# desy-ml/cheetah

Hardware: AMD Instinct MI355X
Metric: particle-element-steps/sec at 1e6 particles, 100-elem linac (higher is better)
Workload: dtype f32; 1 GPU; C2: 100-element Drift+Quadrupole FODO, 1e6 particles per GPU, fp32, element-by-element tracking (no map merging) + global beam moments; elements=100, particles_per_gpu=1000000, parallelism=particle-shard x1, sigma_x_checked=True

## Files before the change

### cheetah_amd/_lib.py

```python

from __future__ import annotations

import ctypes
import os

import torch

_HERE = os.path.dirname(os.path.abspath(__file__))
LIB_PATH = os.path.join(_HERE, "libchx.so")

c_void_p, c_int, c_i64, c_double, c_size_t = (
    ctypes.c_void_p,
    ctypes.c_int,
    ctypes.c_int64,
    ctypes.c_double,
    ctypes.c_size_t,
)
c_i32_p = ctypes.POINTER(ctypes.c_int32)
c_u8_p = ctypes.POINTER(ctypes.c_uint8)
c_vpp = ctypes.POINTER(ctypes.c_void_p)
c_double_p = ctypes.POINTER(ctypes.c_double)


class ChxError(RuntimeError):
# ... 6 lines not shown
        ("ndim", ctypes.c_int32),
        ("cols", ctypes.c_int32 * 3),
        ("bins", ctypes.c_int32 * 3),
        ("grid_strides", ctypes.c_int64 * 3),
        ("grid_batch_stride", ctypes.c_int64),
        ("B", c_i64), ("Bx", c_i64), ("Bq", c_i64), ("Bs", c_i64), ("Be", c_i64),
        ("Bsc", c_i64), ("Bsh", c_i64), ("N", c_i64),
        ("dtype", ctypes.c_int32),
        ("abs_charge", ctypes.c_int32),
        ("x", c_void_p), ("charge", c_void_p), ("survival", c_void_p), ("extent", c_void_p),
        ("scale", c_void_p), ("shift", c_void_p), ("grid", c_void_p),
    ]


class LatticeScreen(ctypes.Structure):

    _fields_ = [
        ("rows", c_void_p), ("charges", c_void_p), ("survival", c_void_p), ("energy", c_void_p), ("s", c_void_p),
        ("image", c_void_p), ("image_bytes", c_i64), ("map", c_void_p), ("element_maps", c_void_p),
        ("mu", c_void_p), ("cov", c_void_p), ("geom", c_void_p), ("shift", c_void_p), ("total_charge", c_void_p),
        ("total_charge_out", c_void_p), ("width", ctypes.c_int32), ("height", ctypes.c_int32),
        ("mom_partials", c_void_p),
    ]


class Hist2dArgs(ctypes.Structure):

    _fields_ = [
        ("B", c_i64), ("Bx", c_i64), ("Bq", c_i64), ("Bs", c_i64), ("Bsh", c_i64), ("N", c_i64),
        ("nx", ctypes.c_int32), ("ny", ctypes.c_int32), ("dtype", ctypes.c_int32),
        ("x", c_void_p), ("charge", c_void_p), ("survival", c_void_p), ("shift", c_void_p),
        ("edges_x", c_void_p), ("edges_y", c_void_p), ("image", c_void_p),
    ]


SIGNATURES = {
    "chx_kind_num_params": (c_int, [c_int]),
    "chx_abi_version": (c_int, []),
    "chx_status_string": (ctypes.c_char_p, [c_int]),
    "chx_build_rmatrix": (c_int, [c_int, c_void_p, c_void_p, c_double, c_double, c_i64, c_i64, c_i64, c_int, c_void_p, c_void_p]),
    "chx_build_rmatrix_vjp": (c_int, [c_int, c_void_p, c_void_p, c_double, c_double, c_void_p, c_i64, c_i64, c_i64, c_int, c_void_p, c_void_p, c_void_p]),
    "chx_compose_maps": (c_int, [c_vpp, c_u8_p, c_i64, c_i64, c_int, c_void_p, c_void_p]),
    "chx_compose_maps_vjp_workspace_bytes": (c_size_t, [c_i64, c_i64]),
    "chx_compose_maps_vjp": (c_int, [c_vpp, c_u8_p, c_i64, c_i64, c_int, c_void_p, c_void_p, c_void_p, c_size_t, c_void_p]),
    "chx_compose_prefix": (c_int, [c_void_p, c_i64, c_i64, c_i64, c_int, c_void_p, c_void_p]),
    "chx_run_state_bytes": (c_size_t, [c_i64]),
    "chx_run_map": (c_int, [c_void_p, c_void_p, c_i64, c_void_p, c_double, c_double, c_int, c_void_p, c_size_t, c_void_p,
                            c_void_p, c_void_p, c_void_p]),
    "chx_run_track": (c_int, [c_void_p, c_void_p, c_i64, c_void_p, c_double, c_double, c_int, c_void_p, c_size_t, c_void_p,
                              c_void_p, c_i64, c_void_p, c_void_p, c_void_p]),
    "chx_apply_affine7": (c_int, [c_void_p, c_void_p, c_void_p, c_i64, c_i64, c_i64, c_i64, c_int, c_void_p]),
    "chx_apply_bwd_workspace_bytes": (c_size_t, [c_i64, c_i64]),
    "chx_apply_affine7_bwd": (c_int, [c_void_p, c_void_p, c_void_p, c_void_p, c_void_p, c_i64, c_i64, c_i64, c_i64, c_int, c_void_p, c_size_t, c_void_p]),
    "chx_track_elementwise": (c_int, [c_void_p, c_void_p, c_void_p, c_void_p, c_i64, c_i64, c_i64, c_i64, c_i64, c_int, c_void_p]),
    "chx_track_fused": (c_int, [c_void_p, c_void_p, c_void_p, c_i64, c_i64, c_i64, c_i64, c_i64, c_int, c_void_p]),
    "chx_cavity_coeffs": (c_int, [c_void_p, c_void_p, c_double, c_double, c_i64, c_i64, c_i64, c_int, c_void_p, c_void_p, c_void_p]),
    "chx_cavity_track": (c_int, [c_void_p, c_void_p, c_void_p, c_void_p, c_i64, c_i64, c_i64, c_int, c_void_p]),
    "chx_cavity_track_bwd": (c_int, [c_void_p, c_void_p, c_void_p, c_void_p, c_void_p, c_i64, c_i64, c_i64, c_int, c_void_p,
                                     c_size_t, c_void_p]),
    "chx_moments_workspace_bytes": (c_size_t, [c_i64, c_i64]),
    "chx_moment_sums": (c_int, [c_void_p, c_void_p, c_i64, c_i64, c_i64, c_i64, c_int, c_void_p, c_void_p, c_size_t, c_void_p]),
    "chx_moment_centred": (c_int, [c_void_p, c_void_p, c_void_p, c_i64, c_i64, c_i64, c_i64, c_int, c_void_p, c_void_p, c_size_t, c_void_p]),
    "chx_moment_finalize": (c_int, [c_void_p, c_void_p, c_i64, c_void_p, c_void_p]),
    "chx_moments": (c_int, [c_void_p, c_void_p, c_i64, c_i64, c_i64, c_i64, c_int, c_void_p, c_void_p, c_size_t, c_void_p]),
    "chx_moments_entry": (c_int, [c_void_p, c_void_p, c_i64, c_i64, c_i64, c_i64, c_int, c_void_p, c_int, c_int, c_void_p, c_void_p,
                                  c_size_t, c_void_p]),
    "chx_moments_bwd": (c_int, [c_void_p, c_void_p, c_void_p, c_void_p, c_i64, c_i64, c_i64, c_i64, c_int, c_void_p, c_void_p]),
    "chx_moments_bwd_w": (c_int, [c_void_p, c_void_p, c_void_p, c_void_p, c_i64, c_i64, c_i64, c_i64, c_int, c_void_p, c_void_p,
                                  c_void_p]),
    "chx_moments_mapped_bwd": (c_int, [c_void_p, c_void_p, c_void_p, c_i64, c_i64, c_i64, c_int, c_void_p, c_void_p]),
    "chx_moment_entry": (c_int, [c_void_p, c_i64, c_int, c_int, c_int, c_void_p, c_void_p]),
    "chx_moment_entry_mapped_bwd": (c_int, [c_void_p, c_void_p, c_int, c_int, c_void_p, c_void_p, c_i64, c_i64, c_i64, c_int,
                                            c_void_p, c_int, c_void_p]),
    "chx_cic_deposit": (c_int, [ctypes.POINTER(CicArgs), c_void_p]),
    "chx_cic_deposit_mapped": (c_int, [ctypes.POINTER(CicArgs), c_void_p, c_i64, c_void_p]),
    "chx_cic_sorted_workspace_bytes": (c_size_t, [ctypes.POINTER(CicArgs)]),
    "chx_cic_deposit_sorted": (c_int, [ctypes.POINTER(CicArgs), c_void_p, c_size_t, c_void_p]),
    "chx_cic_deposit_sorted_overwrite": (c_int, [ctypes.POINTER(CicArgs), c_void_p, c_size_t, c_void_p]),
    "chx_cic_indices": (c_int, [ctypes.POINTER(CicArgs), c_void_p, c_void_p, c_void_p]),
    "chx_cic_deposit_bwd": (c_int, [ctypes.POINTER(CicArgs), c_void_p, c_void_p, c_void_p, c_void_p]),
    "chx_hist2d": (c_int, [ctypes.POINTER(Hist2dArgs), c_void_p]),
    "chx_hist2d_indices": (c_int, [ctypes.POINTER(Hist2dArgs), c_void_p, c_void_p]),
    "chx_sc_igf_workspace_bytes": (c_size_t, [c_i64, c_i32_p]),
    "chx_sc_igf": (c_int, [c_void_p, c_void_p, c_i64, c_i32_p, c_int, c_void_p, c_i64, c_void_p, c_size_t, c_void_p]),
    "chx_sc_igf_from_table": (c_int, [c_void_p, c_i64, c_i32_p, c_int, c_void_p, c_i64, c_void_p]),
    "chx_sc_pruned_supported": (c_int, [c_i32_p, c_int]),
    "chx_sc_igf_table": (c_int, [c_void_p, c_void_p, c_i64, c_i32_p, c_int, c_void_p, c_void_p]),
    "chx_sc_green_workspace_bytes": (c_size_t, [c_i64, c_i32_p, c_int]),
    "chx_sc_green_fast_workspace_bytes": (c_size_t, [c_i64, c_i32_p, c_int]),
    "chx_sc_green_spectrum_fast": (c_int, [c_void_p, c_void_p, c_i64, c_i32_p, c_int, c_void_p, c_void_p, c_size_t, c_void_p]),
    "chx_sc_green_spectrum": (c_int, [c_void_p, c_i64, c_i32_p, c_int, c_void_p, c_void_p, c_size_t, c_void_p]),
    "chx_sc_convolve_workspace_bytes": (c_size_t, [c_i64, c_i32_p, c_int]),
    "chx_sc_convolve": (c_int, [c_void_p, c_void_p, c_void_p, c_i64, c_i32_p, c_int, c_void_p, c_void_p, c_size_t, c_void_p]),
    "chx_sc_fft_plan_create": (c_int, [c_i64, c_i32_p, c_int, c_vpp]),
    "chx_sc_fft_plan_destroy": (c_int, [c_void_p]),
    "chx_sc_fft_exec": (c_int, [c_void_p, c_int, c_void_p, c_void_p]),
    "chx_sc_spectral_mul": (c_int, [c_void_p, c_void_p, c_void_p, c_i64, c_i64, c_int, c_void_p]),
    "chx_sc_phi_halo_elements": (c_size_t, [c_i64, c_i32_p]),
    "chx_sc_convolve_halo": (c_int, [c_void_p, c_void_p, c_void_p, c_i64, c_i32_p, c_int, c_void_p, c_void_p, c_size_t, c_void_p]),
    "chx_sc_convolve_halo_after": (c_int, [c_void_p, c_void_p, c_void_p, c_i64, c_i32_p, c_int, c_void_p, c_void_p, c_size_t, c_void_p,
                                           c_void_p]),
    "chx_sc_gather_kick_phi": (c_int, [c_void_p, c_void_p, c_void_p, c_void_p, c_void_p, c_void_p, c_void_p, c_double, c_i64, c_i64,
                                       c_i64, c_i64, c_i32_p, c_int, c_void_p, c_i64, c_void_p, c_void_p]),
    "chx_sc_gradient": (c_int, [c_void_p, c_void_p, c_void_p, c_i64, c_i32_p, c_int, c_i64, c_int, c_void_p, c_void_p]),
    "chx_sc_gather_kick": (c_int, [c_void_p, c_void_p, c_void_p, c_void_p, c_void_p, c_void_p, c_double, c_i64, c_i64, c_i64, c_i64, c_i32_p, c_int, c_void_p, c_void_p]),
    "chx_sc_gather_kick_mapped": (c_int, [c_void_p, c_void_p, c_void_p, c_void_p, c_void_p, c_void_p, c_double, c_i64, c_i64, c_i64,
# ... 227 lines not shown
```

### cheetah_amd/_ops.py

```python

from __future__ import annotations

import ctypes
import weakref
import os

import torch

from . import _lib
from ._lib import CicArgs, Hist2dArgs, check

KIND = {
    "identity": 0, "drift": 1, "quadrupole": 2, "dipole": 3, "hcor": 4, "vcor": 5, "ccor": 6,
    "cavity_sw": 7, "cavity_tw": 8, "solenoid": 9, "undulator": 10,
}
NUM_PARAMS = [0, 1, 5, 9, 2, 2, 3, 4, 4, 4, 4]
MOM_NOUT = 29
CAV_NCOEF = 8


def dtype_code(dtype: torch.dtype) -> int:
    if dtype == torch.float32:
        return 0
    if dtype == torch.float64:
# ... 461 lines not shown
    root = _origin(source)
    copy._chx_origin = (weakref.ref(root), root._version, copy._version)


def _origin(t: torch.Tensor) -> torch.Tensor:
    while True:
        tag = getattr(t, "_chx_origin", None)
        if tag is None or tag[2] != t._version:
            return t
        src = tag[0]()
        if src is None or src._version != tag[1]:
            return t
        t = src


def apply_map(particles: torch.Tensor, tm: torch.Tensor) -> torch.Tensor:
    require_device(particles, tm)
    if tm.dtype != particles.dtype:
        raise RuntimeError(f"transfer map dtype {tm.dtype} does not match particle dtype {particles.dtype}")
    N = particles.shape[-2]
    batch_shape = bshapes(particles.shape[:-2], tm.shape[:-2])
    B = numel(batch_shape)
    x, _ = flat_bcast(particles, batch_shape, 2)
    R, _ = flat_bcast(tm, batch_shape, 2)
    x, R = aligned(x), R.contiguous()
    if x.requires_grad or R.requires_grad:
        out = Apply.apply(x, R, B).reshape(*batch_shape, N, 7)
        if not x.requires_grad and torch.is_grad_enabled():
            out._chx_lin = _LinearSource(_origin(particles), x, R, batch_shape, out._version)
        return out
    out = _apply_raw(x, R, B, x.shape[0], R.shape[0], N)
    return out.reshape(*batch_shape, N, 7)


def track_elementwise(particles, maps: torch.Tensor, fused: bool = False) -> torch.Tensor:
    require_device(particles, maps)
    if torch.is_grad_enabled() and (particles.requires_grad or maps.requires_grad):
        x = particles
        for e in range(maps.shape[0]):
            x = apply_map(x, maps[e] if maps.shape[1] > 1 else maps[e, 0])
        return x
    E, BR = maps.shape[0], maps.shape[1]
    N = particles.shape[-2]
    batch_shape = torch.broadcast_shapes(particles.shape[:-2], (BR,) if BR > 1 else ())
    B = numel(batch_shape)
    x, Bx = flat_bcast(particles, batch_shape, 2)
    x, maps = aligned(x), maps.contiguous()
    out = torch.empty((B, N, 7), dtype=x.dtype, device=x.device)
    lib = _lib.lib()
    if fused:
        check(lib.chx_track_fused(ptr(x), ptr(maps), ptr(out), E, B, Bx, BR, N, dtype_code(x.dtype), stream_ptr()),
              "chx_track_fused")
    else:
        check(lib.chx_track_elementwise(ptr(x), ptr(maps), ptr(out), None, E, B, Bx, BR, N,
                                        dtype_code(x.dtype), stream_ptr()), "chx_track_elementwise")
    return out.reshape(*batch_shape, N, 7)


def _cavity_coeffs_autograd(params, energy, mass_eV, n_charges, B):
    import math

    p = params.to(torch.float64).expand(B, 4)
    L, V, phi, freq = p[:, 0], p[:, 1], p[:, 2] * (math.pi / 180.0), p[:, 3]
    E0 = energy.to(torch.float64).expand(B)
    g0 = E0 / mass_eV
    ig2 = 1.0 / (g0 * g0)
    b0 = (1.0 - ig2).sqrt()
    cphi, sphi = phi.cos(), phi.sin()
    dEn = V * cphi * n_charges * -1.0
    E1 = E0 + dEn
    g1 = E1 / mass_eV
    b1 = (1.0 - 1.0 / (g1 * g1)).sqrt()
    k = 2.0 * math.pi * freq / 299792458.0
    gain = (dEn > 0).any()
    dg = V / mass_eV
    b03, b13, g03, g13 = b0**3, b1**3, g0**3, g1**3
    gd = g0 - g1
    gd = torch.where(gd == 0, torch.ones_like(gd), gd)
    T566_gain = L * (b03 * g03 - b13 * g13) / (2.0 * b0 * b13 * g0 * gd * g13)
    T556_gain = b0 * k * L * dg * g0 * (b13 * g13 + b0 * (g0 - g13)) * sphi / (b13 * g13 * gd * gd)
    T555_gain = b0 * b0 * k * k * L * dg / 2.0 * (
        dg * (2.0 * g0 * g13 * (b0 * b13 - 1.0) + g0 * g0 + 3.0 * g1 * g1 - 2.0) / (b13 * g13 * gd**3) * sphi * sphi
        - (g1 * g0 * (b1 * b0 - 1.0) + 1.0) / (b1 * g1 * gd * gd) * cphi)
    zero = torch.zeros_like(L)
    T566 = torch.where(gain, T566_gain, 1.5 * L * ig2 / b03)
    T556 = torch.where(gain, T556_gain, zero)
    T555 = torch.where(gain, T555_gain, zero)
    coeffs = torch.stack([E0 * b0 / (E1 * b1), V * b0 / (E1 * b1), b0 * k, phi, cphi, T566, T556, T555], dim=-1)
    return coeffs, E1.to(energy.dtype)


def cavity_coeffs(params, energy, mass_eV, n_charges, B):
    if params.requires_grad or energy.requires_grad:
        return _cavity_coeffs_autograd(params, energy, mass_eV, n_charges, B)
    coeffs = torch.empty((B, CAV_NCOEF), dtype=torch.float64, device=energy.device)
    e_out = torch.empty((B,), dtype=energy.dtype, device=energy.device)
    check(_lib.lib().chx_cavity_coeffs(ptr(params), ptr(energy), mass_eV, n_charges, B, params.shape[0],
                                       energy.shape[0], dtype_code(energy.dtype), ptr(coeffs), ptr(e_out),
                                       stream_ptr()), "chx_cavity_coeffs")
    return coeffs, e_out


def _cavity_track_raw(x, R, coeffs, B, N):
    out = torch.empty((B, N, 7), dtype=x.dtype, device=x.device)
    check(_lib.lib().chx_cavity_track(ptr(x), ptr(R), ptr(coeffs), ptr(out), B, x.shape[0], N,
                                      dtype_code(x.dtype), stream_ptr()), "chx_cavity_track")
    return out
# ... 753 lines not shown
```

### cheetah_amd/csrc/chx_apply.hip

```cpp
#include <cstdlib>
#include <type_traits>

#include "chx_common.h"
#include "chx_apply_tiles.h"
#include "chx_cic_dev.h"

namespace {

template <typename T> __device__ __forceinline__ T chx_fma(T a, T b, T c);
template <> __device__ __forceinline__ float chx_fma<float>(float a, float b, float c) { return fmaf(a, b, c); }
template <> __device__ __forceinline__ double chx_fma<double>(double a, double b, double c) { return fma(a, b, c); }

template <typename T>
__device__ __forceinline__ void apply7(const T* __restrict__ R, const T (&x)[7], T (&y)[7]) {
#pragma unroll
    for (int i = 0; i < 7; ++i) {
        T acc = R[i * 7] * x[0];
#pragma unroll
        for (int j = 1; j < 7; ++j) acc = chx_fma<T>(R[i * 7 + j], x[j], acc);
        y[i] = acc;
    }
}

template <typename T>
// ... 409 lines not shown
        int64_t wchunks = (8192 + wtiles - 1) / wtiles;
        if (wchunks > B) wchunks = B;
        int64_t wrows = (B + wchunks - 1) / wchunks;
        if (wrows < 8 && B >= 8) wrows = 8;
        wchunks = (B + wrows - 1) / wrows;
        if (wtiles > 0x7fffffffLL || wchunks > 65535) return CHX_ERR_INVALID_ARG;
        hipLaunchKernelGGL((apply_shared_wave_kernel<T, WPPT>), dim3((unsigned)wtiles, (unsigned)wchunks), dim3(CHX_BLOCK), 0, s,
                           (const T*)x_in, (const T*)R, (T*)x_out, B, N, wrows, (int)chx_aligned16(x_in));
    } else
        hipLaunchKernelGGL((apply_shared_kernel<T, PPT>), dim3((unsigned)tiles, (unsigned)chunks),
                           dim3(CHX_BLOCK), 0, s, (const T*)x_in, (const T*)R, (T*)x_out, B, N, rows,
                           (int)chx_aligned16(x_in), (int)chx_aligned16(x_out));
    CHX_CHECK_LAUNCH();
    return CHX_OK;
}

int check_common(const void* x_in, const void* R, const void* x_out, int64_t B, int64_t Bx,
                 int64_t BR, int64_t N, int dtype) {
    if (!x_in || !R || !x_out || B < 1 || N < 1) return CHX_ERR_INVALID_ARG;
    if (!chx_bcast_ok(Bx, B) || !chx_bcast_ok(BR, B)) return CHX_ERR_INVALID_ARG;
    if (dtype != CHX_F32 && dtype != CHX_F64) return CHX_ERR_DTYPE;
    const size_t esz = dtype == CHX_F32 ? 4 : 8;
    if ((reinterpret_cast<uintptr_t>(x_in) % esz) || (reinterpret_cast<uintptr_t>(x_out) % esz) ||
        (reinterpret_cast<uintptr_t>(R) % esz))
        return CHX_ERR_MISALIGNED;
    return CHX_OK;
}

}

extern "C" int chx_apply_affine7(const void* x_in, const void* R, void* x_out, int64_t B, int64_t Bx,
                                 int64_t BR, int64_t N, int dtype, void* stream) {
    int st = check_common(x_in, R, x_out, B, Bx, BR, N, dtype);
    if (st != CHX_OK) return st;
    hipStream_t s = (hipStream_t)stream;
    if (Bx == 1 && B > 1 && BR == B) {
        return dtype == CHX_F32 ? launch_shared<float>(x_in, R, x_out, B, N, s)
                                : launch_shared<double>(x_in, R, x_out, B, N, s);
    }
    return dtype == CHX_F32 ? launch_tiles<float, 0>(x_in, R, x_out, nullptr, B, Bx, BR, N, 1, s)
                            : launch_tiles<double, 0>(x_in, R, x_out, nullptr, B, Bx, BR, N, 1, s);
}

extern "C" int chx_track_fused(const void* x_in, const void* R, void* x_out, int64_t E, int64_t B,
                               int64_t Bx, int64_t BR, int64_t N, int dtype, void* stream) {
    int st = check_common(x_in, R, x_out, B, Bx, BR, N, dtype);
    if (st != CHX_OK) return st;
    if (E < 1 || E > 0x7fffffff) return CHX_ERR_INVALID_ARG;
    hipStream_t s = (hipStream_t)stream;
    return dtype == CHX_F32 ? launch_tiles<float, 1>(x_in, R, x_out, nullptr, B, Bx, BR, N, (int)E, s)
                            : launch_tiles<double, 1>(x_in, R, x_out, nullptr, B, Bx, BR, N, (int)E, s);
}

extern "C" int chx_track_elementwise(const void* x_in, const void* R, void* x_out, void* scratch,
                                     int64_t E, int64_t B, int64_t Bx, int64_t BR, int64_t N,
                                     int dtype, void* stream) {
    int st = check_common(x_in, R, x_out, B, Bx, BR, N, dtype);
    if (st != CHX_OK) return st;
    if (E < 1) return CHX_ERR_INVALID_ARG;
    const size_t esz = dtype == CHX_F32 ? 4 : 8;
    const char* Rp = (const char*)R;
    (void)scratch;
    st = chx_apply_affine7(x_in, Rp, x_out, B, Bx, BR, N, dtype, stream);
    hipStream_t s = (hipStream_t)stream;
    if (st == CHX_OK && chx_coltile_ok(x_out, E, B, N, dtype)) return chx_coltile_passes(x_out, R, E, B, BR, N, dtype, s);
    for (int64_t e = 1; e < E && st == CHX_OK; ++e) {
        const void* Re = Rp + (size_t)e * (size_t)BR * 49 * esz;
        st = dtype == CHX_F32 ? launch_inplace_pass<float>(x_out, Re, B, BR, N, s)
                              : launch_inplace_pass<double>(x_out, Re, B, BR, N, s);
    }
    return st;
}

extern "C" int chx_cavity_track(const void* x_in, const void* R, const double* coeffs, void* x_out,
                                int64_t B, int64_t Bx, int64_t N, int dtype, void* stream) {
    int st = check_common(x_in, R, x_out, B, Bx, B, N, dtype);
    if (st != CHX_OK) return st;
    if (!coeffs) return CHX_ERR_INVALID_ARG;
    hipStream_t s = (hipStream_t)stream;
    return dtype == CHX_F32 ? launch_tiles<float, 2>(x_in, R, x_out, coeffs, B, Bx, B, N, 1, s)
                            : launch_tiles<double, 2>(x_in, R, x_out, coeffs, B, Bx, B, N, 1, s);
}

extern "C" size_t chx_cavity_track_scalars_workspace_bytes(void) { return 49 * sizeof(double) + 8 + CHX_CAV_NCOEF * sizeof(double); }

extern "C" int chx_cavity_track_scalars(const void* x_in, const void* const* param_ptrs, const void* energy, int kind,
                                        double mass_eV, double n_charges, int64_t N, int dtype, void* x_out, void* energy_out,
                                        const void* s_in, void* s_out, void* workspace, size_t workspace_bytes, void* stream) {
    if (!x_in || !x_out || !workspace || workspace_bytes < chx_cavity_track_scalars_workspace_bytes() || N < 1)
        return CHX_ERR_INVALID_ARG;
    if ((reinterpret_cast<uintptr_t>(workspace) & 7) != 0) return CHX_ERR_MISALIGNED;
    void* R = workspace;
    double* coeffs = reinterpret_cast<double*>((char*)workspace + 49 * sizeof(double) + 8);
    int st = chx_cavity_prepare_scalars(param_ptrs, energy, kind, mass_eV, n_charges, dtype, R, coeffs, energy_out, s_in, s_out,
                                        stream);
    if (st != CHX_OK) return st;
    return chx_cavity_track(x_in, R, coeffs, x_out, 1, 1, N, dtype, stream);
}

namespace {
struct ApplyScreens {
    chx_lattice_screen s[CHX_LATTICE_MAX_SCREENS];
    const void* charge;
};

constexpr int kApplyStagedItems = 96;
constexpr int kMomSlots = 64;
constexpr int kApplyMapStride = 52;

template <typename T, int PPT, int SCREENS, bool STAGED>
__global__ __launch_bounds__(CHX_BLOCK) void lattice_apply_kernel(const T* x_in, T* x_out, const int64_t* __restrict__ items_g, int n_items,
                                                                 const double* __restrict__ Rs, const double* __restrict__ coeffs_g,
                                                                 int64_t N, int in_vec_ok, int out_vec_ok,
                                                                 const T* __restrict__ survival, double* __restrict__ bpm_ws, int diag,
                                                                 const int64_t* __restrict__ ptrs, T* __restrict__ survival_out,
                                                                 int shared_in ,
                                                                 int64_t Bm ,
                                                                 int shared_sv ,
// ... 882 lines not shown
```

### cheetah_amd/csrc/chx_apply_tiles.h

```cpp
#pragma once
#include "chx_common.h"

template <typename T> struct tile_cfg;
template <> struct tile_cfg<float> { static constexpr int PPT = 2; };
template <> struct tile_cfg<double> { static constexpr int PPT = 1; };

constexpr int64_t kSmallBeamBytes = (int64_t)14 * 1024 * 1024 + 700 * 1024;
constexpr int64_t kL2ResidentBytes = (int64_t)28 * 1024 * 1024;
constexpr int64_t kColTileMinBytes = (int64_t)8 * 1024 * 1024;

bool chx_coltile_ok(const void* x, int64_t E, int64_t B, int64_t N, int dtype);
int chx_coltile_passes(void* x, const void* R, int64_t E, int64_t B, int64_t BR, int64_t N, int dtype, hipStream_t s);
```

### cheetah_amd/csrc/chx_coltile.hip

```cpp
#include "chx_common.h"
#include "chx_apply_tiles.h"

namespace {

template <typename T> struct coltile_cfg {
    static constexpr int TP = tile_cfg<T>::PPT * CHX_BLOCK;
    static constexpr int LANES = TP / (16 / (int)sizeof(T));
};

template <typename T, bool TO_COLUMNS>
__global__ __launch_bounds__(CHX_BLOCK) void coltile_edge_kernel(T* x, const T* __restrict__ R, int64_t BR, int64_t N) {
    constexpr int TP = coltile_cfg<T>::TP;
    __shared__ __attribute__((aligned(16))) T lds[TP * 7];
    const int64_t tiles_per_row = (N + TP - 1) / TP;
    const int64_t b = blockIdx.x / tiles_per_row;
    const int64_t n0 = (blockIdx.x - b * tiles_per_row) * TP;
    const int np = (int)((N - n0 < TP) ? (N - n0) : TP);
    chx_coltile_edge<T, TP, TO_COLUMNS>(x + (b * N + n0) * 7, R + ((BR == 1) ? 0 : b) * 49, lds, np, true);
}

template <typename T, bool NT_LOAD>
__global__ __launch_bounds__(coltile_cfg<T>::LANES) void coltile_pass_kernel(T* x, const T* __restrict__ R, int64_t BR, int64_t N) {
    constexpr int TP = coltile_cfg<T>::TP;
    const int64_t tiles_per_row = (N + TP - 1) / TP;
    const int64_t b = blockIdx.x / tiles_per_row;
    const int64_t n0 = (blockIdx.x - b * tiles_per_row) * TP;
    T* g = x + (b * N + n0) * 7;
    const T* __restrict__ Rb = R + ((BR == 1) ? 0 : b) * 49;
    if (N - n0 >= TP) chx_coltile_pass<T, TP, NT_LOAD>(g, Rb);
    else chx_rowtile_pass<T>(g, Rb, (int)(N - n0));
}

template <typename T>
bool coltile_ok(const void* x, int64_t E, int64_t B, int64_t N) {
    const int64_t bytes = B * N * 7 * (int64_t)sizeof(T);
    return E >= 3 && chx_aligned16(x) && (B == 1 || (N * 7 * (int64_t)sizeof(T)) % 16 == 0) &&
           bytes >= kColTileMinBytes;
}

template <typename T>
int launch_coltile_passes(void* x, const void* R, int64_t E, int64_t B, int64_t BR, int64_t N, hipStream_t s) {
    constexpr int TP = coltile_cfg<T>::TP;
    const int64_t tiles = ((N + TP - 1) / TP) * B;
    if (tiles > 0x7fffffffLL) return CHX_ERR_INVALID_ARG;
    const bool nt_load = B * N * 7 * (int64_t)sizeof(T) > kL2ResidentBytes;
    const T* Rp = (const T*)R;
    const int64_t estride = BR * 49;
    hipLaunchKernelGGL((coltile_edge_kernel<T, true>), dim3((unsigned)tiles), dim3(CHX_BLOCK), 0, s, (T*)x, Rp + estride, BR, N);
    for (int64_t e = 2; e < E - 1; ++e) {
        if (nt_load)
            hipLaunchKernelGGL((coltile_pass_kernel<T, true>), dim3((unsigned)tiles), dim3(coltile_cfg<T>::LANES), 0, s, (T*)x,
                               Rp + e * estride, BR, N);
        else
            hipLaunchKernelGGL((coltile_pass_kernel<T, false>), dim3((unsigned)tiles), dim3(coltile_cfg<T>::LANES), 0, s, (T*)x,
                               Rp + e * estride, BR, N);
    }
    hipLaunchKernelGGL((coltile_edge_kernel<T, false>), dim3((unsigned)tiles), dim3(CHX_BLOCK), 0, s, (T*)x, Rp + (E - 1) * estride,
                       BR, N);
    CHX_CHECK_LAUNCH();
    return CHX_OK;
}

}

bool chx_coltile_ok(const void* x, int64_t E, int64_t B, int64_t N, int dtype) {
    return dtype == CHX_F32 ? coltile_ok<float>(x, E, B, N) : coltile_ok<double>(x, E, B, N);
}

int chx_coltile_passes(void* x, const void* R, int64_t E, int64_t B, int64_t BR, int64_t N, int dtype, hipStream_t s) {
    return dtype == CHX_F32 ? launch_coltile_passes<float>(x, R, E, B, BR, N, s) : launch_coltile_passes<double>(x, R, E, B, BR, N, s);
}
```

### cheetah_amd/csrc/chx_common.h

```cpp
#pragma once
#include <hip/hip_runtime.h>
#include <stdint.h>
#include "chx.h"

#define CHX_WAVE 64
#define CHX_BLOCK 256

#define CHX_CHECK_LAUNCH()                                   \
    do {                                                     \
        hipError_t e__ = hipGetLastError();                  \
        if (e__ != hipSuccess) return CHX_ERR_LAUNCH;        \
    } while (0)

static inline bool chx_bcast_ok(int64_t b, int64_t B) { return b == 1 || b == B; }
static __host__ __device__ inline bool chx_aligned16(const void* p) { return (reinterpret_cast<uintptr_t>(p) & 15u) == 0; }

template <typename T> struct chx_vec16;
template <> struct chx_vec16<float> { using type = float4; static constexpr int n = 4; };
template <> struct chx_vec16<double> { using type = double2; static constexpr int n = 2; };

template <int CTRL>
__device__ __forceinline__ double chx_dpp_add(double v) {
    const int lo = __double2loint(v), hi = __double2hiint(v);
    const int lo2 = __builtin_amdgcn_update_dpp(0, lo, CTRL, 0xf, 0xf, true);
// ... 212 lines not shown
    const int lane = threadIdx.x & 63;
    if (vec_ok) {
        const int nvec = n_elem / VN;
        const V* __restrict__ gv = reinterpret_cast<const V*>(g);
        V* lv = reinterpret_cast<V*>(wl);
        if (nt) {
            for (int v = lane; v < nvec; v += 64) lv[v] = chx_nt_load(gv + v);
        } else {
            for (int v = lane; v < nvec; v += 64) lv[v] = gv[v];
        }
        for (int e = nvec * VN + lane; e < n_elem; e += 64) wl[e] = g[e];
    } else {
        for (int e = lane; e < n_elem; e += 64) wl[e] = g[e];
    }
}

template <typename T>
__device__ __forceinline__ void wave_tile_store(T* __restrict__ g, const T* __restrict__ wl, int n_elem, bool vec_ok,
                                                 bool nt = false) {
    using V = typename chx_vec16<T>::type;
    constexpr int VN = chx_vec16<T>::n;
    const int lane = threadIdx.x & 63;
    if (vec_ok) {
        const int nvec = n_elem / VN;
        V* __restrict__ gv = reinterpret_cast<V*>(g);
        const V* lv = reinterpret_cast<const V*>(wl);
        if (nt) {
            for (int v = lane; v < nvec; v += 64) chx_nt_store(lv[v], gv + v);
        } else {
            for (int v = lane; v < nvec; v += 64) gv[v] = lv[v];
        }
        for (int e = nvec * VN + lane; e < n_elem; e += 64) g[e] = wl[e];
    } else {
        for (int e = lane; e < n_elem; e += 64) g[e] = wl[e];
    }
}

typedef unsigned chx_v4u __attribute__((ext_vector_type(4)));
template <typename T> struct chx_col16;
template <> struct chx_col16<float> { using V = chx_v4f; using P = chx_v2f; };
template <> struct chx_col16<double> { using V = chx_v2d; using P = chx_v2d; };

template <typename T, typename X>
__device__ __forceinline__ void chx_map7(const T* __restrict__ R, const X (&x)[7], X (&y)[7]) {
#pragma unroll
    for (int i = 0; i < 7; ++i) {
        X acc = x[0] * R[i * 7];
#pragma unroll
        for (int j = 1; j < 7; ++j) acc = __builtin_elementwise_fma((X)R[i * 7 + j], x[j], acc);
        y[i] = acc;
    }
}

template <typename T, int TP, bool NT_LOAD, bool NT_STORE = true>
__device__ __forceinline__ void chx_coltile_pass(T* g, const T* __restrict__ R) {
    using V = typename chx_col16<T>::V;
    using P = typename chx_col16<T>::P;
    constexpr int LANES = TP / (16 / (int)sizeof(T));
    V* gv = reinterpret_cast<V*>(g) + threadIdx.x;
    V x[7], y[7];
#pragma unroll
    for (int j = 0; j < 7; ++j) x[j] = NT_LOAD ? __builtin_nontemporal_load(gv + j * LANES) : gv[j * LANES];
    if constexpr (sizeof(T) == 4) {
        P lo[7], hi[7], ylo[7], yhi[7];
#pragma unroll
        for (int j = 0; j < 7; ++j) { lo[j] = x[j].xy; hi[j] = x[j].zw; }
        chx_map7<T, P>(R, lo, ylo);
        chx_map7<T, P>(R, hi, yhi);
#pragma unroll
        for (int j = 0; j < 7; ++j) { y[j].xy = ylo[j]; y[j].zw = yhi[j]; }
    } else {
        chx_map7<T, P>(R, x, y);
    }
#pragma unroll
    for (int j = 0; j < 7; ++j) {
        const chx_v4u d = __builtin_bit_cast(chx_v4u, y[j]) ^ __builtin_bit_cast(chx_v4u, x[j]);
        if (__any((d.x | d.y | d.z | d.w) != 0u)) {
            if (NT_STORE) __builtin_nontemporal_store(y[j], gv + j * LANES);
            else gv[j * LANES] = y[j];
        }
    }
}

template <typename T>
__device__ __forceinline__ void chx_rowtile_pass(T* g, const T* __restrict__ R, int np) {
    for (int p = threadIdx.x; p < np; p += blockDim.x) {
        T x[7], y[7];
#pragma unroll
        for (int j = 0; j < 7; ++j) x[j] = g[p * 7 + j];
        chx_map7<T, T>(R, x, y);
#pragma unroll
        for (int j = 0; j < 7; ++j) g[p * 7 + j] = y[j];
    }
}

template <typename T, int TP, bool TO_COLUMNS>
__device__ __forceinline__ void chx_coltile_edge(T* g, const T* __restrict__ R, T* lds, int np, bool vec_ok) {
    constexpr int PPT = TP / CHX_BLOCK;
    const bool full = np == TP;
    const bool in_cols = full && !TO_COLUMNS, out_cols = full && TO_COLUMNS;
    tile_load<T, TP>(g, lds, np * 7, vec_ok, false);
    __syncthreads();
    T y[PPT][7];
#pragma unroll
    for (int k = 0; k < PPT; ++k) {
        const int p = threadIdx.x + k * CHX_BLOCK;
        if (p < np) {
            T x[7];
#pragma unroll
            for (int j = 0; j < 7; ++j) x[j] = in_cols ? lds[j * TP + p] : lds[p * 7 + j];
            chx_map7<T, T>(R, x, y[k]);
        }
    }
    if (full) __syncthreads();
#pragma unroll
    for (int k = 0; k < PPT; ++k) {
        const int p = threadIdx.x + k * CHX_BLOCK;
        if (p < np) {
#pragma unroll
            for (int j = 0; j < 7; ++j) lds[out_cols ? j * TP + p : p * 7 + j] = y[k][j];
        }
    }
    __syncthreads();
    tile_store<T, TP>(g, lds, np * 7, vec_ok, true);
}

static inline int chx_grid_for(int64_t work_items, int per_block, int cap) {
    int64_t g = (work_items + per_block - 1) / per_block;
    if (g < 1) g = 1;
    if (g > cap) g = cap;
    return (int)g;
}
```

### include/chx.h

```cpp
#ifndef CHX_H
#define CHX_H

#include <stddef.h>
#include <stdint.h>

#ifdef __cplusplus
extern "C" {
#endif

#define CHX_ABI_VERSION 9

typedef enum chx_status {
    CHX_OK = 0,
    CHX_ERR_INVALID_ARG = -1,
    CHX_ERR_DTYPE = -2,
    CHX_ERR_MISALIGNED = -3,
    CHX_ERR_LAUNCH = -4,
    CHX_ERR_WORKSPACE = -5,
    CHX_ERR_NO_DEVICE = -6
} chx_status;

typedef enum chx_dtype { CHX_F32 = 0, CHX_F64 = 1 } chx_dtype;

typedef enum chx_kind {
// ... 16 lines not shown
int chx_abi_version(void);
const char* chx_status_string(int status);

int chx_build_rmatrix(int kind, const void* params, const void* energy, double mass_eV,
                      double n_charges, int64_t B, int64_t Bp, int64_t Be, int dtype,
                      void* R_out, void* stream);

int chx_build_rmatrix_vjp(int kind, const void* params, const void* energy, double mass_eV,
                          double n_charges, const void* dR, int64_t B, int64_t Bp, int64_t Be,
                          int dtype, void* dparams, void* denergy, void* stream);

int chx_build_rmatrix_scalars(const int32_t* kinds, const void* const* param_ptrs, int64_t E, const void* energy,
                              double mass_eV, double n_charges, int dtype, void* R_out, void* stream);
int chx_compose_prefix(const void* maps, int64_t E, int64_t B, int64_t Bm, int dtype, void* out, void* stream);
size_t chx_run_vjp_workspace_bytes(int64_t E);
int chx_run_vjp(const int32_t* kinds, const void* const* param_ptrs, int64_t E, const void* energy, double mass_eV,
                double n_charges, int dtype, const void* maps, const void* dT, void* dinputs, void* workspace,
                size_t workspace_bytes, void* stream);
int chx_run_vjp_masked(const int32_t* kinds, const void* const* param_ptrs, int64_t E, const void* energy, double mass_eV,
                       double n_charges, int dtype, const void* maps, const void* dT, const uint16_t* need, void* dinputs,
                       void* workspace, size_t workspace_bytes, void* stream);
size_t chx_run_vjp_entry_workspace_bytes(int64_t E);
int chx_run_vjp_entry(const int32_t* kinds, const void* const* param_ptrs, int64_t E, const void* energy, double mass_eV,
                      double n_charges, int dtype, const void* maps, const uint16_t* need, const void* grad, const double* mom_y,
                      int index, int take_sqrt, const void* C, const double* mom_x, void* dinputs, void* workspace,
                      size_t workspace_bytes, void* stream);
size_t chx_run_map_batched_workspace_bytes(int64_t E, int64_t B, int dtype);
int chx_run_map_batched(const int32_t* kinds, const void* const* param_ptrs, const uint8_t* batched, int64_t E, int64_t B,
                        const void* energy, int energy_rows, double mass_eV, double n_charges, int dtype, void* workspace,
                        size_t workspace_bytes, void* R_out, void* stream);
int chx_run_build_compose(const int32_t* kinds, const void* const* param_ptrs, int64_t E, const void* energy, double mass_eV,
                          double n_charges, int dtype, void* maps, void* R_out, void* stream);
size_t chx_run_state_bytes(int64_t E);
int chx_run_map(const int32_t* kinds, const void* const* param_ptrs, int64_t E, const void* energy, double mass_eV,
                double n_charges, int dtype, void* state, size_t state_bytes, void** R_out, const void* s_in, void* s_out,
                void* stream);
int chx_run_track(const int32_t* kinds, const void* const* param_ptrs, int64_t E, const void* energy, double mass_eV,
                  double n_charges, int dtype, void* state, size_t state_bytes, const void* x_in, void* x_out, int64_t N,
                  const void* s_in, void* s_out, void* stream);
int chx_compose_maps(const void* const* R_ptrs, const uint8_t* bcast, int64_t E, int64_t B,
                     int dtype, void* R_out, void* stream);
size_t chx_compose_maps_vjp_workspace_bytes(int64_t E, int64_t B);
int chx_compose_maps_vjp(const void* const* R_ptrs, const uint8_t* bcast, int64_t E, int64_t B, int dtype, const void* dT, void* dM,
                         void* workspace, size_t workspace_bytes, void* stream);

int chx_apply_affine7(const void* x_in, const void* R, void* x_out, int64_t B, int64_t Bx,
                      int64_t BR, int64_t N, int dtype, void* stream);

size_t chx_apply_bwd_workspace_bytes(int64_t B, int64_t N);
int chx_apply_affine7_bwd(const void* dY, const void* R, const void* X, void* dX, double* dR,
                          int64_t B, int64_t Bx, int64_t BR, int64_t N, int dtype,
                          void* workspace, size_t workspace_bytes, void* stream);

int chx_track_elementwise(const void* x_in, const void* R , void* x_out,
                          void* scratch, int64_t E, int64_t B, int64_t Bx, int64_t BR,
                          int64_t N, int dtype, void* stream);

int chx_track_fused(const void* x_in, const void* R , void* x_out, int64_t E,
                    int64_t B, int64_t Bx, int64_t BR, int64_t N, int dtype, void* stream);

#define CHX_CAV_NCOEF 8
int chx_cavity_coeffs(const void* params , const void* energy , double mass_eV,
                      double n_charges, int64_t B, int64_t Bp, int64_t Be, int dtype,
                      double* coeffs , void* energy_out ,
                      void* stream);
int chx_cavity_track(const void* x_in, const void* R, const double* coeffs, void* x_out,
                     int64_t B, int64_t Bx, int64_t N, int dtype, void* stream);

int chx_cavity_track_bwd(const void* dY, const void* X, const double* coeffs, void* dX, double* dcoeffs, int64_t B,
                         int64_t Bx, int64_t N, int dtype, void* workspace, size_t workspace_bytes, void* stream);

#define CHX_MOM_NSUMS 8
#define CHX_MOM_NM2 21
#define CHX_MOM_NOUT 29
size_t chx_moments_workspace_bytes(int64_t B, int64_t N);
int chx_moment_sums(const void* x, const void* w, int64_t B, int64_t Bx, int64_t Bw, int64_t N,
                    int dtype, double* sums, void* workspace, size_t workspace_bytes, void* stream);
int chx_moment_centred(const void* x, const void* w, const double* sums, int64_t B, int64_t Bx,
                       int64_t Bw, int64_t N, int dtype, double* m2, void* workspace,
                       size_t workspace_bytes, void* stream);
int chx_moment_finalize(const double* sums, const double* m2, int64_t B, double* out, void* stream);
int chx_moments(const void* x, const void* w, int64_t B, int64_t Bx, int64_t Bw, int64_t N,
                int dtype, double* out, void* workspace, size_t workspace_bytes, void* stream);
int chx_moments_entry(const void* x, const void* w, int64_t B, int64_t Bx, int64_t Bw, int64_t N, int dtype, double* out,
                      int index, int take_sqrt, void* entry_out, void* workspace, size_t workspace_bytes, void* stream);
int chx_merge_moments(const double* per_rank, int32_t R, int64_t B, double* out, void* stream);
int chx_moments_bwd(const void* x, const void* w, const double* out, const double* d_out,
                    int64_t B, int64_t Bx, int64_t Bw, int64_t N, int dtype, void* dX, void* stream);
int chx_moments_bwd_w(const void* x, const void* w, const double* out, const double* d_out, int64_t B, int64_t Bx, int64_t Bw,
                      int64_t N, int dtype, void* dX, void* dW, void* stream);
#define CHX_SLICES_MAX 2048
size_t chx_slice_moments_workspace_bytes(int64_t B, int64_t N, int32_t S);
int chx_slice_moments(const void* x, const void* w, const void* q, const void* edges, int64_t B, int64_t Bx, int64_t Bw, int64_t Bq,
                      int64_t Be, int64_t N, int32_t S, int dtype, double* out, double* charge, void* workspace,
                      size_t workspace_bytes, void* stream);
int chx_slice_moments_bwd(const void* x, const void* w, const void* q, const void* edges, int64_t B, int64_t Bx, int64_t Bw,
                          int64_t Bq, int64_t Be, int64_t N, int32_t S, int dtype, const double* out, const double* d_out,
                          const double* d_charge, void* dX, void* dW, void* dQ, void* workspace, size_t workspace_bytes,
                          void* stream);
#define CHX_WAKE_MAX_BINS 4096
#define CHX_WAKE_STATE_HEADER 8
#define CHX_WAKE_STATE_DOUBLES(M) (CHX_WAKE_STATE_HEADER + 6 * (int64_t)(M))
size_t chx_wake_workspace_bytes(int64_t B, int64_t N, int32_t M);
int chx_wake_kick(const void* x, const void* q, const void* w, const double* scale, const double* wl, int64_t Ll, const double* wt,
                  int64_t Lt, const double* h, int64_t B, int64_t Bx, int64_t Bq, int64_t Bw, int64_t N, int32_t M, int dtype,
                  void* out, double* state, void* workspace, size_t workspace_bytes, void* stream);
// ... 336 lines not shown
```

Before: 191.4 billion particle-element-steps/s.

## Skip reloading constant-one column in coltile passes via per-tile flags

Adds a per-tile flag buffer, allocated as scratch from Python, that records whether column 6 (the homogeneous coordinate) of each tile is all ones after the entry pass. Later in-place passes read the flag and, when it is set, substitute a constant one instead of loading column 6 from memory. This cuts global reads per pass by roughly one seventh. Any pass that writes a changed column 6 clears the flag. The cost is an extra scratch allocation per call, a flag load per tile, and branchy flag logic that must stay consistent across passes.

```diff
diff --git a/cheetah_amd/_lib.py b/cheetah_amd/_lib.py
--- a/cheetah_amd/_lib.py
+++ b/cheetah_amd/_lib.py
@@ -82,6 +82,7 @@
     "chx_apply_affine7": (c_int, [c_void_p, c_void_p, c_void_p, c_i64, c_i64, c_i64, c_i64, c_int, c_void_p]),
     "chx_apply_bwd_workspace_bytes": (c_size_t, [c_i64, c_i64]),
     "chx_apply_affine7_bwd": (c_int, [c_void_p, c_void_p, c_void_p, c_void_p, c_void_p, c_i64, c_i64, c_i64, c_i64, c_int, c_void_p, c_size_t, c_void_p]),
+    "chx_track_elementwise_scratch_bytes": (c_size_t, [c_i64, c_i64, c_int]),
     "chx_track_elementwise": (c_int, [c_void_p, c_void_p, c_void_p, c_void_p, c_i64, c_i64, c_i64, c_i64, c_i64, c_int, c_void_p]),
     "chx_track_fused": (c_int, [c_void_p, c_void_p, c_void_p, c_i64, c_i64, c_i64, c_i64, c_i64, c_int, c_void_p]),
     "chx_cavity_coeffs": (c_int, [c_void_p, c_void_p, c_double, c_double, c_i64, c_i64, c_i64, c_int, c_void_p, c_void_p, c_void_p]),
diff --git a/cheetah_amd/_ops.py b/cheetah_amd/_ops.py
--- a/cheetah_amd/_ops.py
+++ b/cheetah_amd/_ops.py
@@ -537,7 +537,9 @@
         check(lib.chx_track_fused(ptr(x), ptr(maps), ptr(out), E, B, Bx, BR, N, dtype_code(x.dtype), stream_ptr()),
               "chx_track_fused")
     else:
-        check(lib.chx_track_elementwise(ptr(x), ptr(maps), ptr(out), None, E, B, Bx, BR, N,
+        nbytes = lib.chx_track_elementwise_scratch_bytes(B, N, dtype_code(x.dtype))
+        scratch = torch.empty(nbytes, dtype=torch.uint8, device=x.device) if nbytes else None
+        check(lib.chx_track_elementwise(ptr(x), ptr(maps), ptr(out), ptr(scratch) if nbytes else None, E, B, Bx, BR, N,
                                         dtype_code(x.dtype), stream_ptr()), "chx_track_elementwise")
     return out.reshape(*batch_shape, N, 7)
 
diff --git a/cheetah_amd/csrc/chx_apply.hip b/cheetah_amd/csrc/chx_apply.hip
--- a/cheetah_amd/csrc/chx_apply.hip
+++ b/cheetah_amd/csrc/chx_apply.hip
@@ -485,18 +485,23 @@
                             : launch_tiles<double, 1>(x_in, R, x_out, nullptr, B, Bx, BR, N, (int)E, s);
 }
 
+extern "C" size_t chx_track_elementwise_scratch_bytes(int64_t B, int64_t N, int dtype) {
+    if (dtype != CHX_F32 && dtype != CHX_F64) return 0;
+    return chx_coltile_scratch_bytes(B, N, dtype);
+}
+
 extern "C" int chx_track_elementwise(const void* x_in, const void* R, void* x_out, void* scratch,
                                      int64_t E, int64_t B, int64_t Bx, int64_t BR, int64_t N,
                                      int dtype, void* stream) {
     int st = check_common(x_in, R, x_out, B, Bx, BR, N, dtype);
     if (st != CHX_OK) return st;
     if (E < 1) return CHX_ERR_INVALID_ARG;
+    if (reinterpret_cast<uintptr_t>(scratch) % sizeof(unsigned)) return CHX_ERR_MISALIGNED;
     const size_t esz = dtype == CHX_F32 ? 4 : 8;
     const char* Rp = (const char*)R;
-    (void)scratch;
     st = chx_apply_affine7(x_in, Rp, x_out, B, Bx, BR, N, dtype, stream);
     hipStream_t s = (hipStream_t)stream;
-    if (st == CHX_OK && chx_coltile_ok(x_out, E, B, N, dtype)) return chx_coltile_passes(x_out, R, E, B, BR, N, dtype, s);
+    if (st == CHX_OK && chx_coltile_ok(x_out, E, B, N, dtype)) return chx_coltile_passes(x_out, R, scratch, E, B, BR, N, dtype, s);
     for (int64_t e = 1; e < E && st == CHX_OK; ++e) {
         const void* Re = Rp + (size_t)e * (size_t)BR * 49 * esz;
         st = dtype == CHX_F32 ? launch_inplace_pass<float>(x_out, Re, B, BR, N, s)
diff --git a/cheetah_amd/csrc/chx_apply_tiles.h b/cheetah_amd/csrc/chx_apply_tiles.h
--- a/cheetah_amd/csrc/chx_apply_tiles.h
+++ b/cheetah_amd/csrc/chx_apply_tiles.h
@@ -9,5 +9,7 @@
 constexpr int64_t kL2ResidentBytes = (int64_t)28 * 1024 * 1024;
 constexpr int64_t kColTileMinBytes = (int64_t)8 * 1024 * 1024;
 
+
 bool chx_coltile_ok(const void* x, int64_t E, int64_t B, int64_t N, int dtype);
-int chx_coltile_passes(void* x, const void* R, int64_t E, int64_t B, int64_t BR, int64_t N, int dtype, hipStream_t s);
+size_t chx_coltile_scratch_bytes(int64_t B, int64_t N, int dtype);
+int chx_coltile_passes(void* x, const void* R, void* flags, int64_t E, int64_t B, int64_t BR, int64_t N, int dtype, hipStream_t s);
diff --git a/cheetah_amd/csrc/chx_coltile.hip b/cheetah_amd/csrc/chx_coltile.hip
--- a/cheetah_amd/csrc/chx_coltile.hip
+++ b/cheetah_amd/csrc/chx_coltile.hip
@@ -31,6 +31,31 @@
     else chx_rowtile_pass<T>(g, Rb, (int)(N - n0));
 }
 
+template <typename T, bool NT_LOAD>
+__global__ __launch_bounds__(coltile_cfg<T>::LANES) void coltile_pass_flag_kernel(T* x, const T* __restrict__ R, unsigned* flags,
+                                                                                  int64_t N, int64_t BR) {
+    constexpr int TP = coltile_cfg<T>::TP;
+    const int64_t tiles_per_row = (N + TP - 1) / TP;
+    const int64_t b = blockIdx.x / tiles_per_row;
+    const int64_t n0 = (blockIdx.x - b * tiles_per_row) * TP;
+    T* g = x + (b * N + n0) * 7;
+    const T* __restrict__ Rb = R + ((BR == 1) ? 0 : b) * 49;
+    if (N - n0 >= TP) chx_coltile_pass<T, TP, NT_LOAD, true, true>(g, Rb, flags + blockIdx.x);
+    else chx_rowtile_pass<T>(g, Rb, (int)(N - n0));
+}
+
+template <typename T>
+__global__ __launch_bounds__(CHX_BLOCK) void coltile_enter_kernel(T* x, const T* __restrict__ R, unsigned* flags, int64_t N, int64_t BR) {
+    constexpr int TP = coltile_cfg<T>::TP;
+    __shared__ __attribute__((aligned(16))) T lds[TP * 7];
+    const int64_t tiles_per_row = (N + TP - 1) / TP;
+    const int64_t b = blockIdx.x / tiles_per_row;
+    const int64_t n0 = (blockIdx.x - b * tiles_per_row) * TP;
+    const int np = (int)((N - n0 < TP) ? (N - n0) : TP);
+    T* g = x + (b * N + n0) * 7;
+    chx_coltile_enter<T, TP>(g, g, R + ((BR == 1) ? 0 : b) * 49, lds, np, true, false, flags + blockIdx.x);
+}
+
 template <typename T>
 bool coltile_ok(const void* x, int64_t E, int64_t B, int64_t N) {
     const int64_t bytes = B * N * 7 * (int64_t)sizeof(T);
@@ -39,24 +64,33 @@
 }
 
 template <typename T>
-int launch_coltile_passes(void* x, const void* R, int64_t E, int64_t B, int64_t BR, int64_t N, hipStream_t s) {
+size_t coltile_scratch_bytes(int64_t B, int64_t N) {
+    if (B < 1 || N < 1 || B * N * 7 * (int64_t)sizeof(T) < kColTileMinBytes) return 0;
+    constexpr int TP = coltile_cfg<T>::TP;
+    return (size_t)(((N + TP - 1) / TP) * B) * sizeof(unsigned);
+}
+
+template <typename T>
+int launch_coltile_passes(void* x, const void* R, unsigned* flags, int64_t E, int64_t B, int64_t BR, int64_t N, hipStream_t s) {
     constexpr int TP = coltile_cfg<T>::TP;
     const int64_t tiles = ((N + TP - 1) / TP) * B;
     if (tiles > 0x7fffffffLL) return CHX_ERR_INVALID_ARG;
     const bool nt_load = B * N * 7 * (int64_t)sizeof(T) > kL2ResidentBytes;
     const T* Rp = (const T*)R;
     const int64_t estride = BR * 49;
-    hipLaunchKernelGGL((coltile_edge_kernel<T, true>), dim3((unsigned)tiles), dim3(CHX_BLOCK), 0, s, (T*)x, Rp + estride, BR, N);
+    const dim3 grid((unsigned)tiles), lanes(coltile_cfg<T>::LANES);
+    if (flags) hipLaunchKernelGGL((coltile_enter_kernel<T>), grid, dim3(CHX_BLOCK), 0, s, (T*)x, Rp + estride, flags, N, BR);
+    else hipLaunchKernelGGL((coltile_edge_kernel<T, true>), grid, dim3(CHX_BLOCK), 0, s, (T*)x, Rp + estride, BR, N);
     for (int64_t e = 2; e < E - 1; ++e) {
-        if (nt_load)
-            hipLaunchKernelGGL((coltile_pass_kernel<T, true>), dim3((unsigned)tiles), dim3(coltile_cfg<T>::LANES), 0, s, (T*)x,
-                               Rp + e * estride, BR, N);
-        else
-            hipLaunchKernelGGL((coltile_pass_kernel<T, false>), dim3((unsigned)tiles), dim3(coltile_cfg<T>::LANES), 0, s, (T*)x,
-                               Rp + e * estride, BR, N);
+        if (flags) {
+            if (nt_load) hipLaunchKernelGGL((coltile_pass_flag_kernel<T, true>), grid, lanes, 0, s, (T*)x, Rp + e * estride, flags, N, BR);
+            else hipLaunchKernelGGL((coltile_pass_flag_kernel<T, false>), grid, lanes, 0, s, (T*)x, Rp + e * estride, flags, N, BR);
+        } else {
+            if (nt_load) hipLaunchKernelGGL((coltile_pass_kernel<T, true>), grid, lanes, 0, s, (T*)x, Rp + e * estride, BR, N);
+            else hipLaunchKernelGGL((coltile_pass_kernel<T, false>), grid, lanes, 0, s, (T*)x, Rp + e * estride, BR, N);
+        }
     }
-    hipLaunchKernelGGL((coltile_edge_kernel<T, false>), dim3((unsigned)tiles), dim3(CHX_BLOCK), 0, s, (T*)x, Rp + (E - 1) * estride,
-                       BR, N);
+    hipLaunchKernelGGL((coltile_edge_kernel<T, false>), grid, dim3(CHX_BLOCK), 0, s, (T*)x, Rp + (E - 1) * estride, BR, N);
     CHX_CHECK_LAUNCH();
     return CHX_OK;
 }
@@ -67,6 +101,11 @@
     return dtype == CHX_F32 ? coltile_ok<float>(x, E, B, N) : coltile_ok<double>(x, E, B, N);
 }
 
-int chx_coltile_passes(void* x, const void* R, int64_t E, int64_t B, int64_t BR, int64_t N, int dtype, hipStream_t s) {
-    return dtype == CHX_F32 ? launch_coltile_passes<float>(x, R, E, B, BR, N, s) : launch_coltile_passes<double>(x, R, E, B, BR, N, s);
+size_t chx_coltile_scratch_bytes(int64_t B, int64_t N, int dtype) {
+    return dtype == CHX_F32 ? coltile_scratch_bytes<float>(B, N) : coltile_scratch_bytes<double>(B, N);
 }
+
+int chx_coltile_passes(void* x, const void* R, void* flags, int64_t E, int64_t B, int64_t BR, int64_t N, int dtype, hipStream_t s) {
+    return dtype == CHX_F32 ? launch_coltile_passes<float>(x, R, (unsigned*)flags, E, B, BR, N, s)
+                            : launch_coltile_passes<double>(x, R, (unsigned*)flags, E, B, BR, N, s);
+}
diff --git a/cheetah_amd/csrc/chx_common.h b/cheetah_amd/csrc/chx_common.h
--- a/cheetah_amd/csrc/chx_common.h
+++ b/cheetah_amd/csrc/chx_common.h
@@ -288,15 +288,24 @@
     }
 }
 
-template <typename T, int TP, bool NT_LOAD, bool NT_STORE = true>
-__device__ __forceinline__ void chx_coltile_pass(T* g, const T* __restrict__ R) {
+template <typename T, int TP, bool NT_LOAD, bool NT_STORE = true, bool FLAGGED = false>
+__device__ __forceinline__ void chx_coltile_pass(T* g, const T* __restrict__ R, unsigned* flag = nullptr) {
     using V = typename chx_col16<T>::V;
     using P = typename chx_col16<T>::P;
     constexpr int LANES = TP / (16 / (int)sizeof(T));
+    constexpr int NLOAD = FLAGGED ? 6 : 7;
     V* gv = reinterpret_cast<V*>(g) + threadIdx.x;
     V x[7], y[7];
 #pragma unroll
-    for (int j = 0; j < 7; ++j) x[j] = NT_LOAD ? __builtin_nontemporal_load(gv + j * LANES) : gv[j * LANES];
+    for (int j = 0; j < NLOAD; ++j) x[j] = NT_LOAD ? __builtin_nontemporal_load(gv + j * LANES) : gv[j * LANES];
+    unsigned flagged = 0;
+    if constexpr (FLAGGED) {
+        flagged = *flag;
+        T one = (T)1;
+        asm("" : "+v"(one));
+        x[6] = (V)one;
+        if (!flagged) x[6] = NT_LOAD ? __builtin_nontemporal_load(gv + 6 * LANES) : gv[6 * LANES];
+    }
     if constexpr (sizeof(T) == 4) {
         P lo[7], hi[7], ylo[7], yhi[7];
 #pragma unroll
@@ -314,6 +323,7 @@
         if (__any((d.x | d.y | d.z | d.w) != 0u)) {
             if (NT_STORE) __builtin_nontemporal_store(y[j], gv + j * LANES);
             else gv[j * LANES] = y[j];
+            if (FLAGGED && j == 6 && flagged && (threadIdx.x & 63) == 0) *flag = 0u;
         }
     }
 }
@@ -361,6 +371,53 @@
     tile_store<T, TP>(g, lds, np * 7, vec_ok, true);
 }
 
+template <typename T, int TP>
+__device__ __forceinline__ void chx_coltile_enter(const T* gin, T* gout, const T* __restrict__ R, T* lds, int np, bool in_vec,
+                                                  bool nt_in, unsigned* flag) {
+    using V = typename chx_col16<T>::V;
+    constexpr int PPT = TP / CHX_BLOCK;
+    const bool full = np == TP;
+    tile_load<T, TP>(gin, lds, np * 7, in_vec, nt_in);
+    __syncthreads();
+    T y[PPT][7];
+#pragma unroll
+    for (int k = 0; k < PPT; ++k) {
+        const int p = threadIdx.x + k * CHX_BLOCK;
+        if (p < np) {
+            T x[7];
+#pragma unroll
+            for (int j = 0; j < 7; ++j) x[j] = lds[p * 7 + j];
+            chx_map7<T, T>(R, x, y[k]);
+        }
+    }
+    if (full) __syncthreads();
+#pragma unroll
+    for (int k = 0; k < PPT; ++k) {
+        const int p = threadIdx.x + k * CHX_BLOCK;
+        if (p < np) {
+#pragma unroll
+            for (int j = 0; j < 7; ++j) lds[full ? j * TP + p : p * 7 + j] = y[k][j];
+        }
+    }
+    __syncthreads();
+    tile_store<T, TP>(gout, lds, np * 7, true, true);
+    if (threadIdx.x < 64) {
+        bool ones = full;
+        if (full) {
+            constexpr int NV = TP * (int)sizeof(T) / 16 / 64;
+            const V* c6 = reinterpret_cast<const V*>(lds + 6 * TP);
+            const V one = (V)(T)1;
+#pragma unroll
+            for (int i = 0; i < NV; ++i) {
+                const chx_v4u d = __builtin_bit_cast(chx_v4u, c6[threadIdx.x + i * 64]) ^ __builtin_bit_cast(chx_v4u, one);
+                ones = ones && (d.x | d.y | d.z | d.w) == 0u;
+            }
+        }
+        const bool all_ones = __all(ones);
+        if (threadIdx.x == 0) *flag = all_ones ? 1u : 0u;
+    }
+}
+
 static inline int chx_grid_for(int64_t work_items, int per_block, int cap) {
     int64_t g = (work_items + per_block - 1) / per_block;
     if (g < 1) g = 1;
diff --git a/include/chx.h b/include/chx.h
--- a/include/chx.h
+++ b/include/chx.h
@@ -92,6 +92,7 @@
                           int64_t B, int64_t Bx, int64_t BR, int64_t N, int dtype,
                           void* workspace, size_t workspace_bytes, void* stream);
 
+size_t chx_track_elementwise_scratch_bytes(int64_t B, int64_t N, int dtype);
 int chx_track_elementwise(const void* x_in, const void* R , void* x_out,
                           void* scratch, int64_t E, int64_t B, int64_t Bx, int64_t BR,
                           int64_t N, int dtype, void* stream);
```

Measured after the change: 200.8 billion particle-element-steps/s (median of 6 runs). 1.05x the previous value.
